# snap-research/3dgp

Hardware: AMD Instinct MI355X
Metric: generator-forward img/s @256^2, 64 steps (higher is better)
Workload: dtype f32; 1 GPU; BASELINE configs[2]: ImageNet 256x256, 64(+64) ray steps, cmax 512, c_dim 1000, tri-plane 512^2 x 96, full HIP path; batch_per_gpu=16, global_batch=16, img_resolution=256, num_ray_steps=64, depth_adaptor=False, parallelism=dp1 (batch-sharded, weights replicated)

## Files before the change

### 3dgp_amd/csrc/sampling.hip

```cpp
#include "common.h"

namespace {

constexpr int MAXS = 256;
constexpr int RAYS_PER_BLOCK = 4;
constexpr int MAXS_PASS = 512;
constexpr int MAXS_LONG = 1024;

template <int MS>
struct alignas(16) WaveScratchT {
    float z[MS];
    float sig[MS];
    float w[MS + 4];
    float cdf[MS];
    float bins[MS];
    float col[3][MS];
};
using WaveScratch = WaveScratchT<MAXS>;

template <int MS> struct alignas(16) MarchScratchT { float z[MS]; float sig[MS]; float w[MS + 4]; };
template <> struct alignas(16) MarchScratchT<MAXS> : WaveScratch {};
template <int MS> struct alignas(16) UnifyScratchT { float z[MS]; };
template <> struct alignas(16) UnifyScratchT<MAXS> : WaveScratch {};

__device__ __forceinline__ void wave_sync() {
    __builtin_amdgcn_fence(__ATOMIC_ACQ_REL, "wavefront");
    __builtin_amdgcn_wave_barrier();
}

__device__ __forceinline__ float s2t(float s, float t_near, float t_far) { return s * t_far + (1.0f - s) * t_near; }

template <bool LONGX>
__device__ __forceinline__ float exp_neg(float x) { return LONGX ? (float)exp(-(double)x) : expf(-x); }

template <bool LONGX = false>
__device__ void march_classical_lds(const float* z, const float* sig, float* w, int S, int flags, float cut_thr, float& final_T, float& wagg) {
    const int l = lane_id();
    double carry = 1.0;
    float wsum = 0.0f;
    if (S > 64 && S <= 128) {
        float alpha[2], fac[2];
#pragma unroll
        for (int c = 0; c < 2; c++) {
            const int i = 64 * c + l;
            alpha[c] = 0.f; fac[c] = 1.0f;
            if (i < S) {
                const float delta = (i < S - 1) ? (z[i + 1] - z[i]) : ((flags & 1) ? 1e10f : 1e-3f);
                float sp = (flags & 8) ? (sig[i] > 0.f ? sig[i] : 0.f) : softplus20f(sig[i]);
                if (sp < cut_thr) sp = 0.f;
                alpha[c] = 1.0f - exp_neg<LONGX>(delta * sp);
                fac[c] = (1.0f - alpha[c]) + 1e-10f;
            }
        }
        const double s0 = wave_scan_f64<true>((double)fac[0]), s1 = wave_scan_f64<true>((double)fac[1]);
        const double c1 = wave_last_f64(s0);
        const double i1 = s1 * c1;
        const float incl0 = (float)s0, incl1 = (float)i1;
        const float wi0 = alpha[0] * wave_shr1_f32(incl0, 1.0f), wi1 = alpha[1] * wave_shr1_f32(incl1, (float)c1);
        w[l] = wi0; wsum += wi0;
        if (64 + l < S) { w[64 + l] = wi1; wsum += wi1; }
        carry = wave_last_f64(i1);
    } else
    for (int base = 0; base < S; base += 64) {
        const int i = base + l;
        float alpha = 0.f, fac = 1.0f;
        if (i < S) {
            float delta = (i < S - 1) ? (z[i + 1] - z[i]) : ((flags & 1) ? 1e10f : 1e-3f);
            float sp = (flags & 8) ? (sig[i] > 0.f ? sig[i] : 0.f) : softplus20f(sig[i]);
            if (sp < cut_thr) sp = 0.f;
            alpha = 1.0f - exp_neg<LONGX>(delta * sp);
            fac = (1.0f - alpha) + 1e-10f;
        }
        const double incl64 = wave_scan_f64<true>((double)fac) * carry;
        const float incl = (float)incl64;
        const float excl = wave_shr1_f32(incl, (float)carry);
        const float wi = alpha * excl;
        if (i < S) { w[i] = wi; wsum += wi; }
        carry = wave_last_f64(incl64);
    }
    wagg = wave_sum_f32(wsum);
    final_T = (float)carry;
    wave_sync();
    if ((flags & 2) && l == 0) w[S - 1] += (1.0f - wagg);
    wave_sync();
}

template <bool LONGX = false>
__device__ void march_mip_lds(const float* z, const float* sig, float* w, int S, int flags, float density_bias, float cut_thr, float& final_T,
                              float& wagg) {
    const int l = lane_id();
    const int M = (flags & 1) ? S : S - 1;
    double carry = 1.0;
    float wsum = 0.0f;
    for (int base = 0; base < M; base += 64) {
        const int i = base + l;
        float alpha = 0.f, fac = 1.0f;
        if (i < M) {
            float delta, smid;
            if (i < S - 1) { delta = z[i + 1] - z[i]; smid = (sig[i] + sig[i + 1]) / 2.f; }
            else { delta = 1e10f; smid = sig[S - 1]; }
            float sp = softplus20f(smid + density_bias);
            if (sp < cut_thr) sp = 0.f;
            float dd = sp * delta;
            alpha = 1.0f - exp_neg<LONGX>(dd);
            fac = (1.0f - alpha) + 1e-10f;
        }
        const double incl64 = wave_scan_f64<true>((double)fac) * carry;
        const float incl = (float)incl64;
        const float excl = wave_shr1_f32(incl, (float)carry);
        const float wi = alpha * excl;
        if (i < M) { w[i] = wi; wsum += wi; }
        carry = wave_last_f64(incl64);
    }
    wagg = wave_sum_f32(wsum);
    final_T = (float)carry;
    wave_sync();
}

__device__ float torch_order_sum_lds(const float* w1, int n, float eps) {
    const int l = lane_id();
    if (n >= 8) {
        const int nv = n >> 3, nilp = nv >> 2;
        const int col = l & 7, a = (l >> 3) & 3;
        float acc = 0.f;
        for (int i = 0; i < nilp; i++) acc = __fadd_rn(acc, __fadd_rn(w1[(4 * i + a) * 8 + col], eps));
        for (int j = 4 * nilp; j < nv; j++) {
            const float v = __fadd_rn(w1[j * 8 + col], eps);
            if (a == 0) acc = __fadd_rn(acc, v);
        }
        float p = __shfl(acc, col, 64);
        p = __fadd_rn(p, __shfl(acc, col + 8, 64));
        p = __fadd_rn(p, __shfl(acc, col + 16, 64));
        p = __fadd_rn(p, __shfl(acc, col + 24, 64));
        float fin = 0.f;
        for (int k = nv * 8; k < n; k++) fin = __fadd_rn(fin, __fadd_rn(w1[k], eps));
#pragma unroll
        for (int c = 0; c < 8; c++) fin = __fadd_rn(fin, __int_as_float(__builtin_amdgcn_readlane(__float_as_int(p), c)));
        return fin;
    }
    float acc[4] = {0.f, 0.f, 0.f, 0.f};
    const int nilp = n >> 2;
    if (nilp)
        for (int k = 0; k < 4; k++) acc[k] = __fadd_rn(acc[k], __fadd_rn(w1[k], eps));
    for (int r = 4 * nilp; r < n; r++) acc[0] = __fadd_rn(acc[0], __fadd_rn(w1[r], eps));
    for (int k = 1; k < 4; k++) acc[0] = __fadd_rn(acc[0], acc[k]);
    return acc[0];
}

template <typename SC, typename GetU, typename Emit>
__device__ void importance_lds(SC& sc, int S, int Wn, GetU getu, int N, int mip, Emit emit) {
    const int l = lane_id();
    const float eps = 1e-5f;
    float* w = sc.w;
    constexpr int CAP = sizeof(sc.z) / sizeof(float), NV = (CAP > MAXS ? CAP : MAXS) / 64;
    if (mip) {
        float nv[NV];
#pragma unroll
        for (int c = 0; c < NV; c++) {
            const int i = l + 64 * c;
            if (i < Wn) {
                float a = (i - 1 >= 0) ? w[i - 1] : -INFINITY, b = w[i], d = (i + 1 < Wn) ? w[i + 1] : -INFINITY;
                float t0 = a > b ? a : b;
                float t1 = b > d ? b : d;
                nv[c] = (t0 + t1) / 2.f + 0.01f;
            }
        }
        wave_sync();
#pragma unroll
        for (int c = 0; c < NV; c++) {
            const int i = l + 64 * c;
            if (i < Wn) w[i] = nv[c];
        }
    } else {
        for (int i = l; i < Wn; i += 64) w[i] = w[i] + 1e-5f;
    }
    wave_sync();
    const int nb = S - 1, ns = Wn - 2, nc = ns + 1;
    for (int i = l; i < nb; i += 64) sc.bins[i] = 0.5f * (sc.z[i] + sc.z[i + 1]);
    const float totf = torch_order_sum_lds(w + 1, ns, eps);
    double carry = 0.0;
    if (l == 0) sc.cdf[0] = 0.f;
    for (int base = 0; base < ns; base += 64) {
        const int i = base + l;
        float pdf = (i < ns) ? (w[1 + i] + eps) / totf : 0.f;
        double incl = wave_scan_f64<false>((double)pdf) + carry;
        if (i < ns) sc.cdf[i + 1] = (float)incl;
        carry = wave_last_f64(incl);
    }
    wave_sync();
    for (int j = l; j < N; j += 64) {
        const float uu = getu(j);
        int lo = 0, hi = nc;
        while (lo < hi) {
            int mid = (lo + hi) >> 1;
            if (sc.cdf[mid] <= uu) lo = mid + 1; else hi = mid;
        }
        const int ind = lo;
        const int below = ind - 1 < 0 ? 0 : ind - 1;
        const int above = ind > ns ? ns : ind;
        const float cb = sc.cdf[below], ca = sc.cdf[above];
        const float bb = sc.bins[below < nb ? below : nb - 1], ba = sc.bins[above < nb ? above : nb - 1];
        float denom = ca - cb;
        if (denom < eps) denom = 1.f;
        const float smp = bb + (uu - cb) / denom * (ba - bb);
        emit(j, smp, ind, below, above);
    }
}

__device__ __forceinline__ float strat_one(float u, int k, int S, float step, int marcher) {
    auto lin = [&](int q) { return (S == 1) ? 0.f : ((q < S / 2) ? __fmaf_rn(step, (float)q, 0.f) : __fmaf_rn(-step, (float)(S - 1 - q), 1.f)); };
    if (marcher == 0) {
        const float lower = (k == 0) ? lin(0) : 0.5f * (lin(k) + lin(k - 1));
        const float upper = (k == S - 1) ? lin(S - 1) : 0.5f * (lin(k + 1) + lin(k));
        return lower + (upper - lower) * u;
    }
    const float delta = (float)((1.0 - 0.0) / (double)(S - 1));
    return lin(k) + u * delta;
}

__global__ __launch_bounds__(256) void stratified_kernel(const float* __restrict__ u, float* __restrict__ sdist, float* __restrict__ tdist,
                                                        int64_t n, int S, int marcher, float t_near, float t_far) {
    const float step = (1.f - 0.f) / (float)(S - 1);
    for (int64_t i = blockIdx.x * (int64_t)blockDim.x + threadIdx.x; i < n; i += (int64_t)gridDim.x * blockDim.x) {
        const float s = strat_one(u[i], (int)(i % S), S, step, marcher);
        sdist[i] = s;
        if (tdist) tdist[i] = s2t(s, t_near, t_far);
    }
}

__global__ __launch_bounds__(256) void stratified4_kernel(const float4* __restrict__ u, float4* __restrict__ sdist, float4* __restrict__ tdist,
                                                         int64_t n4, int S, int marcher, float t_near, float t_far) {
    const float step = (1.f - 0.f) / (float)(S - 1);
    const int S4 = S >> 2;
    for (int64_t i = blockIdx.x * (int64_t)blockDim.x + threadIdx.x; i < n4; i += (int64_t)gridDim.x * blockDim.x) {
        const int k = (int)(i % S4) * 4;
        const float4 uu = u[i];
        const float4 s = make_float4(strat_one(uu.x, k, S, step, marcher), strat_one(uu.y, k + 1, S, step, marcher), strat_one(uu.z, k + 2, S, step, marcher),
                                     strat_one(uu.w, k + 3, S, step, marcher));
        sdist[i] = s;
        if (tdist) tdist[i] = make_float4(s2t(s.x, t_near, t_far), s2t(s.y, t_near, t_far), s2t(s.z, t_near, t_far), s2t(s.w, t_near, t_far));
    }
}

__global__ __launch_bounds__(256) void density_activation_kernel(const float* __restrict__ x, float* __restrict__ y, int64_t n, int relu, float bias) {
    for (int64_t i = blockIdx.x * (int64_t)blockDim.x + threadIdx.x; i < n; i += (int64_t)gridDim.x * blockDim.x)
        y[i] = relu ? (x[i] > 0.f ? x[i] : 0.f) : softplus20f(x[i] + bias);
}

template <int MS>
__global__ __launch_bounds__(256) void ray_march_kernel(const float* __restrict__ colors, const float* __restrict__ dens,
                                                       const float* __restrict__ depths, float* __restrict__ rgb, float* __restrict__ depth_o,
                                                       float* __restrict__ weights, float* __restrict__ final_T, int64_t rays, int S, int C,
                                                       int marcher, int flags, float density_bias, float cut_thr) {
    __shared__ MarchScratchT<MS> scratch[RAYS_PER_BLOCK];
    const int wv = threadIdx.x >> 6, l = lane_id();
    const int64_t r = (int64_t)blockIdx.x * RAYS_PER_BLOCK + wv;
    if (r >= rays) return;
    MarchScratchT<MS>& sc = scratch[wv];
    for (int i = l; i < S; i += 64) { sc.z[i] = depths[r * S + i]; sc.sig[i] = dens[r * S + i]; }
    wave_sync();
    float fT, wagg;
    const int M = (marcher == 0) ? S : ((flags & 1) ? S : S - 1);
    if (MS > MAXS && S > MAXS) {
        if (marcher == 0) march_classical_lds<(MS > MAXS)>(sc.z, sc.sig, sc.w, S, flags, cut_thr, fT, wagg);
        else march_mip_lds<(MS > MAXS)>(sc.z, sc.sig, sc.w, S, flags, density_bias, cut_thr, fT, wagg);
    } else
    if (marcher == 0) march_classical_lds(sc.z, sc.sig, sc.w, S, flags, cut_thr, fT, wagg);
    else march_mip_lds(sc.z, sc.sig, sc.w, S, flags, density_bias, cut_thr, fT, wagg);
    if (weights) for (int i = l; i < M; i += 64) weights[r * M + i] = sc.w[i];
    for (int c = 0; c <= C; c++) {
        float acc = 0.0f;
        for (int i = l; i < M; i += 64) {
            float v;
            if (c < C) {
                v = colors[(r * S + i) * C + c];
                if (marcher == 1 && i < S - 1) v = (v + colors[(r * S + i + 1) * C + c]) / 2.f;
            } else {
                v = sc.z[i];
                if (marcher == 1 && i < S - 1) v = (v + sc.z[i + 1]) / 2.f;
            }
            acc += sc.w[i] * v;
        }
        float out = wave_sum_f32(acc);
        if (marcher == 1 && c < C) {
            if (flags & 4) out = out + 1.0f - wagg;
            out = out * 2.0f - 1.0f;
        }
        if (l == 0) { if (c < C) rgb[r * C + c] = out; else depth_o[r] = out; }
    }
    if (l == 0) final_T[r] = fT;
}

template <int MS>
__global__ __launch_bounds__(256) void sample_importance_kernel(const float* __restrict__ z, const float* __restrict__ weights,
                                                               const float* __restrict__ u, float* __restrict__ samples, int32_t* __restrict__ inds,
                                                               int32_t* __restrict__ below, int32_t* __restrict__ above, float* __restrict__ cdf_o,
                                                               int64_t rays, int S, int Wn, int N, int mip) {
    __shared__ WaveScratchT<MS> scratch[RAYS_PER_BLOCK];
    const int wv = threadIdx.x >> 6, l = lane_id();
    const int64_t r = (int64_t)blockIdx.x * RAYS_PER_BLOCK + wv;
    if (r >= rays) return;
    WaveScratchT<MS>& sc = scratch[wv];
    for (int i = l; i < S; i += 64) sc.z[i] = z[r * S + i];
    for (int i = l; i < Wn; i += 64) sc.w[i] = weights[r * Wn + i];
    wave_sync();
    importance_lds(sc, S, Wn, [&](int j) { return u[r * N + j]; }, N, mip, [&](int j, float smp, int ind, int bl, int ab) {
        samples[r * N + j] = smp;
        if (inds) { inds[r * N + j] = ind; below[r * N + j] = bl; above[r * N + j] = ab; }
    });
    if (cdf_o) for (int i = l; i < Wn - 1; i += 64) cdf_o[r * (Wn - 1) + i] = sc.cdf[i];
}

template <int NS>
__device__ __forceinline__ void stable_ranks_n(const float* key, int M, int* rank) {
    const int l = lane_id();
    float k[NS];
#pragma unroll
    for (int c = 0; c < NS; c++) { const int i = l + 64 * c; k[c] = i < M ? key[i] : 0.f; rank[c] = 0; }
#pragma unroll 4
    for (int m = 0; m < M; m++) {
        const float km = key[m];
#pragma unroll
        for (int c = 0; c < NS; c++) {
            const int i = l + 64 * c;
            rank[c] += (km < k[c] || (km == k[c] && m < i)) ? 1 : 0;
        }
    }
}
__device__ __forceinline__ void stable_ranks(const float* key, int M, int* rank ) {
#pragma unroll
    for (int c = 0; c < MAXS / 64; c++) rank[c] = 0;
    if (M <= 64) stable_ranks_n<1>(key, M, rank);
    else if (M <= 128) stable_ranks_n<2>(key, M, rank);
    else if (M <= 192) stable_ranks_n<3>(key, M, rank);
    else stable_ranks_n<4>(key, M, rank);
}

template <int NR>
__device__ __forceinline__ void stable_ranks_long(const float* key, int M, int (&rank)[NR]) {
    static_assert(NR == MAXS_PASS / 64 || NR == MAXS_LONG / 64, "stable_ranks_long: 8 or 16 slots");
#pragma unroll
    for (int c = 0; c < NR; c++) rank[c] = 0;
    if (M <= MAXS_PASS) stable_ranks_n<MAXS_PASS / 64>(key, M, rank);
    else stable_ranks_n<NR>(key, M, rank);
}

template <int NS, int CAP>
__device__ __forceinline__ void wave_bitonic_sort_n(float (&key)[CAP], int (&idx)[CAP]) {
    static_assert(NS <= CAP && (NS & (NS - 1)) == 0, "wave_bitonic_sort_n: NS a power of two within the arrays");
    const int l = lane_id();
#pragma unroll
    for (int k = 2; k <= 64 * NS; k <<= 1) {
#pragma unroll
        for (int j = k >> 1; j > 0; j >>= 1) {
            if (j >= 64) {
                const int js = j >> 6;
#pragma unroll
                for (int c = 0; c < NS; c++) {
                    if (c & js) continue;
                    const int c2 = c | js;
                    const bool asc = ((64 * c) & k) == 0;
                    const bool less2 = key[c2] < key[c] || (key[c2] == key[c] && idx[c2] < idx[c]);
                    if (less2 == asc) { const float tk = key[c]; key[c] = key[c2]; key[c2] = tk; const int ti = idx[c]; idx[c] = idx[c2]; idx[c2] = ti; }
                }
            } else {
#pragma unroll
                for (int c = 0; c < NS; c++) {
                    const float pk = __shfl_xor(key[c], j, 64);
                    const int pi = __shfl_xor(idx[c], j, 64);
                    const bool asc = ((64 * c + l) & k) == 0;
                    const bool keep_min = ((l & j) == 0) == asc;
                    const bool partner_less = pk < key[c] || (pk == key[c] && pi < idx[c]);
                    if (partner_less == keep_min) { key[c] = pk; idx[c] = pi; }
                }
            }
        }
    }
}

__device__ __forceinline__ void wave_bitonic_sort(float& key, int& idx) {
    const int l = lane_id();
#pragma unroll
    for (int k = 2; k <= 64; k <<= 1) {
#pragma unroll
        for (int j = k >> 1; j > 0; j >>= 1) {
            const float pk = __shfl_xor(key, j, 64);
            const int pi = __shfl_xor(idx, j, 64);
            const bool keep_min = ((l & j) == 0) == ((l & k) == 0);
            const bool partner_less = pk < key || (pk == key && pi < idx);
            if (partner_less == keep_min) { key = pk; idx = pi; }
        }
    }
}

__device__ __forceinline__ void wave_bitonic_sort2(float (&key)[2], int (&idx)[2]) {
    const int l = lane_id();
#pragma unroll
    for (int k = 2; k <= 128; k <<= 1) {
#pragma unroll
        for (int j = k >> 1; j > 0; j >>= 1) {
            if (j == 64) {
                const bool less1 = key[1] < key[0] || (key[1] == key[0] && idx[1] < idx[0]);
                if (less1) { const float tk = key[0]; key[0] = key[1]; key[1] = tk; const int ti = idx[0]; idx[0] = idx[1]; idx[1] = ti; }
            } else {
#pragma unroll
                for (int c = 0; c < 2; c++) {
                    const float pk = __shfl_xor(key[c], j, 64);
                    const int pi = __shfl_xor(idx[c], j, 64);
                    const bool asc = k == 128 ? true : (k == 64 ? c == 0 : ((l & k) == 0));
                    const bool keep_min = ((l & j) == 0) == asc;
                    const bool partner_less = pk < key[c] || (pk == key[c] && pi < idx[c]);
                    if (partner_less == keep_min) { key[c] = pk; idx[c] = pi; }
                }
            }
        }
    }
}

template <int MS>
__global__ __launch_bounds__(256) void importance_from_coarse_kernel(const float* __restrict__ rgbs, const float* __restrict__ sdist,
                                                                    const float* __restrict__ u_fine, float* __restrict__ tfine,
                                                                    float* __restrict__ sfine, int32_t* __restrict__ inds,
                                                                    int32_t* __restrict__ fine_perm, int64_t rays, int S, int N,
                                                                    int marcher, int flags, float density_bias, float cut_thr, float t_near, float t_far) {
    __shared__ WaveScratchT<MS> scratch[RAYS_PER_BLOCK];
    const int wv = threadIdx.x >> 6, l = lane_id();
    const int64_t r = (int64_t)blockIdx.x * RAYS_PER_BLOCK + wv;
    if (r >= rays) return;
    WaveScratchT<MS>& sc = scratch[wv];
    for (int i = l; i < S; i += 64) { sc.z[i] = sdist[r * S + i]; sc.sig[i] = rgbs[(r * S + i) * 4 + 3]; }
    float upre[MS / 64];
    if constexpr (MS > MAXS) {
        for (int i = l; i < N; i += 64) sc.col[1][i] = u_fine[r * N + i];
    } else {
#pragma unroll
    for (int c = 0; c < MS / 64; c++) upre[c] = (l + 64 * c < N) ? u_fine[r * N + l + 64 * c] : 0.f;
    }
    wave_sync();
    float fT, wagg;
    int Wn = S;
    if (MS > MAXS && S > MAXS) {
        if (marcher == 0) march_classical_lds<(MS > MAXS)>(sc.z, sc.sig, sc.w, S, flags, cut_thr, fT, wagg);
        else { march_mip_lds<(MS > MAXS)>(sc.z, sc.sig, sc.w, S, flags, density_bias, cut_thr, fT, wagg); Wn = (flags & 1) ? S : S - 1; }
    } else
    if (marcher == 0) march_classical_lds(sc.z, sc.sig, sc.w, S, flags, cut_thr, fT, wagg);
    else { march_mip_lds(sc.z, sc.sig, sc.w, S, flags, density_bias, cut_thr, fT, wagg); Wn = (flags & 1) ? S : S - 1; }
    float* tkey = sc.col[0];
    if constexpr (MS > MAXS)
        [[clang::always_inline]] importance_lds(sc, S, Wn, [&](int j) { return sc.col[1][j]; }, N, marcher, [&](int j, float smp, int ind, int, int) {
            tkey[j] = s2t(smp, t_near, t_far);
            if (sfine) sfine[r * N + j] = smp;
            if (inds) inds[r * N + j] = ind;
        });
    else
    importance_lds(sc, S, Wn, [&](int j) { float v = upre[0];
#pragma unroll
                                          for (int c = 1; c < MS / 64; c++) v = (j >> 6) == c ? upre[c] : v;
                                          return v; }, N, marcher, [&](int j, float smp, int ind, int, int) {
        tkey[j] = s2t(smp, t_near, t_far);
        if (sfine) sfine[r * N + j] = smp;
        if (inds) inds[r * N + j] = ind;
    });
    wave_sync();
    if (N <= 64) {
        float key = l < N ? tkey[l] : INFINITY;
        {
            if (l >= N) tkey[l] = INFINITY;
            wave_sync();
            int cnt = 0;
#pragma unroll
            for (int jj = 0; jj < 16; jj++) {
                const float4 k4 = *(const float4*)&tkey[4 * jj];
                cnt += (k4.x < key ? 1 : 0) + (k4.y < key ? 1 : 0) + (k4.z < key ? 1 : 0) + (k4.w < key ? 1 : 0);
            }
            int* slot = (int*)sc.bins;
            if (l < N) slot[cnt] = l;
            wave_sync();
            const bool mine = l >= N || slot[cnt] == l;
            if (__all(mine)) {
                if (l < N) {
                    const int src = slot[l];
                    tfine[r * N + l] = tkey[src];
                    if (fine_perm) fine_perm[r * N + l] = src;
                }
                return;
            }
        }
        int idx = l;
        wave_bitonic_sort(key, idx);
        if (l < N) {
            tfine[r * N + l] = key;
            if (fine_perm) fine_perm[r * N + l] = idx;
        }
        return;
    }
    if (N <= 128) {
        float key[2] = {tkey[l], l + 64 < N ? tkey[l + 64] : INFINITY};
        {
            if (l + 64 >= N) tkey[l + 64] = INFINITY;
            wave_sync();
            int cnt[2] = {0, 0};
#pragma unroll 8
            for (int jj = 0; jj < 32; jj++) {
                const float4 k4 = *(const float4*)&tkey[4 * jj];
#pragma unroll
                for (int c = 0; c < 2; c++)
                    cnt[c] += (k4.x < key[c] ? 1 : 0) + (k4.y < key[c] ? 1 : 0) + (k4.z < key[c] ? 1 : 0) + (k4.w < key[c] ? 1 : 0);
            }
            int* slot = (int*)sc.bins;
            slot[cnt[0]] = l;
            if (l + 64 < N) slot[cnt[1]] = l + 64;
            wave_sync();
            const bool mine = slot[cnt[0]] == l && (l + 64 >= N || slot[cnt[1]] == l + 64);
            if (__all(mine)) {
#pragma unroll
                for (int c = 0; c < 2; c++) {
                    const int pos = l + 64 * c;
                    if (pos < N) {
                        const int src = slot[pos];
                        tfine[r * N + pos] = tkey[src];
                        if (fine_perm) fine_perm[r * N + pos] = src;
                    }
                }
                return;
            }
        }
        int idx[2] = {l, l + 64};
        wave_bitonic_sort2(key, idx);
#pragma unroll
        for (int c = 0; c < 2; c++) {
            const int pos = l + 64 * c;
            if (pos < N) {
                tfine[r * N + pos] = key[c];
                if (fine_perm) fine_perm[r * N + pos] = idx[c];
            }
        }
        return;
    }
    if constexpr (MS > MAXS) {
        constexpr int NSL = MS / 64;
        float key[NSL];
        int idx[NSL];
#pragma unroll
        for (int c = 0; c < NSL; c++) { const int e = l + 64 * c; key[c] = e < N ? tkey[e] : INFINITY; idx[c] = e; }
        if (N <= 256) wave_bitonic_sort_n<4>(key, idx);
        else wave_bitonic_sort_n<NSL>(key, idx);
#pragma unroll
        for (int c = 0; c < NSL; c++) {
            const int pos = l + 64 * c;
            if (pos < N) {
                tfine[r * N + pos] = key[c];
                if (fine_perm) fine_perm[r * N + pos] = idx[c];
            }
        }
        return;
    } else {
    int rank[MAXS / 64];
    stable_ranks(tkey, N, rank);
#pragma unroll
    for (int c = 0; c < MAXS / 64; c++) {
        const int j = l + 64 * c;
        if (j < N) {
            tfine[r * N + rank[c]] = tkey[j];
            if (fine_perm) fine_perm[r * N + rank[c]] = j;
        }
    }
    }
}

template <int MS>
__global__ __launch_bounds__(256) void unify_kernel(const float* __restrict__ d1, const float* __restrict__ c1, const float* __restrict__ s1, int S1,
                                                   const float* __restrict__ d2, const float* __restrict__ c2, const float* __restrict__ s2, int S2,
                                                   float* __restrict__ d, float* __restrict__ c, float* __restrict__ s, int32_t* __restrict__ perm,
                                                   int64_t rays, int C) {
    __shared__ UnifyScratchT<MS> scratch[RAYS_PER_BLOCK];
    const int wv = threadIdx.x >> 6, l = lane_id();
    const int64_t r = (int64_t)blockIdx.x * RAYS_PER_BLOCK + wv;
    if (r >= rays) return;
    UnifyScratchT<MS>& sc = scratch[wv];
    const int M = S1 + S2;
    for (int i = l; i < M; i += 64) sc.z[i] = i < S1 ? d1[r * S1 + i] : d2[r * S2 + (i - S1)];
    wave_sync();
    int rank[MS / 64];
    if constexpr (MS > MAXS) stable_ranks_long(sc.z, M, rank);
    else stable_ranks(sc.z, M, rank);
#pragma unroll
    for (int cc = 0; cc < MS / 64; cc++) {
        const int i = l + 64 * cc;
        if (i >= M) continue;
        const int pos = rank[cc];
        d[r * M + pos] = sc.z[i];
        s[r * M + pos] = i < S1 ? s1[r * S1 + i] : s2[r * S2 + (i - S1)];
        for (int k = 0; k < C; k++) c[(r * M + pos) * C + k] = i < S1 ? c1[(r * S1 + i) * C + k] : c2[(r * S2 + (i - S1)) * C + k];
        if (perm) perm[r * M + pos] = i;
    }
}

template <int MS>
__global__ __launch_bounds__(256) void merge_composite_kernel(const float* __restrict__ rgbs1, const float* __restrict__ t1, int S1,
                                                             const float* __restrict__ rgbs2, const float* __restrict__ t2, int S2,
                                                             float* __restrict__ rgb, float* __restrict__ depth_o, float* __restrict__ wsum_o,
                                                             float* __restrict__ final_T, int32_t* __restrict__ perm, const int32_t* __restrict__ perm2, int64_t rays,
                                                             int marcher, int flags, float density_bias, float cut_thr) {
    __shared__ WaveScratchT<MS> scratch[RAYS_PER_BLOCK];
    const int wv = threadIdx.x >> 6, l = lane_id();
    const int64_t r = (int64_t)blockIdx.x * RAYS_PER_BLOCK + wv;
    if (r >= rays) return;
    WaveScratchT<MS>& sc = scratch[wv];
    const int M = S1 + S2;
    float4 cval[MS / 64];
#pragma unroll
    for (int cc = 0; cc < MS / 64; cc++) {
        const int i = l + 64 * cc;
        if (i < M) {
            sc.cdf[i] = i < S1 ? t1[r * S1 + i] : t2[r * S2 + (i - S1)];
            cval[cc] = i < S1 ? ((const float4*)rgbs1)[r * S1 + i] : ((const float4*)rgbs2)[r * S2 + (i - S1)];
        }
    }
    wave_sync();
    bool bad = false;
    for (int i = l; i < M; i += 64)
        if (i + 1 < M && i + 1 != S1 && sc.cdf[i + 1] < sc.cdf[i]) bad = true;
    constexpr int RK = (MS > MAXS ? MS : MAXS) / 64;
    int rank[RK];
    if (__any(bad)) {
        if constexpr (MS > MAXS) stable_ranks_long(sc.cdf, M, rank);
        else stable_ranks(sc.cdf, M, rank);
    } else {
        constexpr int NSL = MS / 64;
        float v[NSL];
        int lo[NSL], hi[NSL];
        bool fine[NSL];
        int* const last = (int*)sc.bins;
        for (int c = l; c <= S1 && c < MS; c += 64) last[c] = 0;
#pragma unroll
        for (int cc = 0; cc < NSL; cc++) {
            const int i = l + 64 * cc;
            v[cc] = i < M ? sc.cdf[i] : 0.f;
            fine[cc] = i >= S1 && i < M;
            lo[cc] = 0;
            hi[cc] = fine[cc] ? S1 : 0;
        }
        const int steps = 32 - __clz(S1);
        for (int it = 0; it < steps; it++) {
#pragma unroll
            for (int cc = 0; cc < NSL; cc++) {
                if (64 * cc + 64 <= S1) continue;
                const bool open = lo[cc] < hi[cc];
                const int mid = (lo[cc] + hi[cc]) >> 1;
                const float o = sc.cdf[open ? mid : 0];
                const bool right = o <= v[cc];
                lo[cc] = (open && right) ? mid + 1 : lo[cc];
                hi[cc] = (open && !right) ? mid : hi[cc];
            }
        }
        wave_sync();
#pragma unroll
        for (int cc = 0; cc < NSL; cc++) {
            const int i = l + 64 * cc;
            if (fine[cc]) atomicMax(&last[lo[cc]], i - S1 + 1);
        }
        wave_sync();
#pragma unroll
        for (int cc = 0; cc < RK; cc++) rank[cc] = 0;
        int carry = 0;
#pragma unroll
        for (int cc = 0; cc < NSL; cc++) {
            const int i = l + 64 * cc;
            if (64 * cc < S1) {
                const int incl = max(wave_scan_max_i32((i <= S1 && i < MS) ? last[i] : 0), carry);
                carry = wave_last_i32(incl);
                rank[cc] = fine[cc] ? (i - S1) + lo[cc] : i + incl;
            } else {
                rank[cc] = (i - S1) + lo[cc];
            }
        }
    }
#pragma unroll
    for (int cc = 0; cc < MS / 64; cc++) {
        const int i = l + 64 * cc;
        if (i >= M) continue;
        const int pos = rank[cc];
        const float4 v = cval[cc];
        sc.z[pos] = sc.cdf[i];
        sc.col[0][pos] = v.x; sc.col[1][pos] = v.y; sc.col[2][pos] = v.z; sc.sig[pos] = v.w;
        if (perm) perm[r * M + pos] = i < S1 ? i : S1 + (perm2 ? perm2[r * S2 + (i - S1)] : i - S1);
    }
    wave_sync();
    float fT, wagg;
    const int Mm = (marcher == 0) ? M : ((flags & 1) ? M : M - 1);
    if (MS > MAXS && M > MAXS) {
        if (marcher == 0) march_classical_lds<(MS > MAXS)>(sc.z, sc.sig, sc.w, M, flags, cut_thr, fT, wagg);
        else march_mip_lds<(MS > MAXS)>(sc.z, sc.sig, sc.w, M, flags, density_bias, cut_thr, fT, wagg);
    } else
    if (marcher == 0) march_classical_lds(sc.z, sc.sig, sc.w, M, flags, cut_thr, fT, wagg);
    else march_mip_lds(sc.z, sc.sig, sc.w, M, flags, density_bias, cut_thr, fT, wagg);
    float acc[4] = {0.f, 0.f, 0.f, 0.f}, wacc = 0.f;
    for (int i = l; i < Mm; i += 64) {
        const float wi = sc.w[i];
        wacc += wi;
#pragma unroll
        for (int c = 0; c < 4; c++) {
            float v = c < 3 ? sc.col[c][i] : sc.z[i];
            if (marcher == 1 && i < M - 1) v = (v + (c < 3 ? sc.col[c][i + 1] : sc.z[i + 1])) / 2.f;
            acc[c] += wi * v;
        }
    }
    float out[4];
#pragma unroll
    for (int c = 0; c < 4; c++) out[c] = wave_sum_f32(acc[c]);
    const float wtot = wave_sum_f32(wacc);
    if (marcher == 1) {
#pragma unroll
        for (int c = 0; c < 3; c++) {
            if (flags & 4) out[c] = out[c] + 1.0f - wagg;
            out[c] = out[c] * 2.0f - 1.0f;
        }
    }
    if (l == 0) {
        rgb[r * 3 + 0] = out[0]; rgb[r * 3 + 1] = out[1]; rgb[r * 3 + 2] = out[2];
        depth_o[r] = out[3];
        if (wsum_o) wsum_o[r] = wtot;
        if (final_T) final_T[r] = fT;
    }
}

inline int ray_blocks(int64_t rays) { return (int)cdiv64(rays, RAYS_PER_BLOCK); }

}

TDGP_API int tdgp_sample_stratified(const float* u, float* sdist, float* tdist, int64_t rays, int S, int marcher, float t_near,
                                    float t_far, tdgp_stream_t stream) {
    TDGP_CHECK(u && sdist, TDGP_EINVAL, "sample_stratified: null pointer");
    TDGP_CHECK(S >= 2 && rays >= 0, TDGP_EINVAL, "sample_stratified: need S >= 2");
    TDGP_CHECK(marcher == 0 || marcher == 1, TDGP_EINVAL, "sample_stratified: unknown ray marcher %d", marcher);
    const int64_t n = rays * S;
    if (n == 0) return TDGP_OK;
    if ((S & 3) == 0 && (((uintptr_t)u | (uintptr_t)sdist | (uintptr_t)tdist) & 15) == 0) {
        TDGP_LAUNCH("stratified_kernel", stratified4_kernel, dim3((int)min((int64_t)8192, cdiv64(n / 4, 256))), dim3(256), 0, (hipStream_t)stream, (const float4*)u,
                    (float4*)sdist, (float4*)tdist, n / 4, S, marcher, t_near, t_far);
        TDGP_LAUNCH_CHECK();
        return TDGP_OK;
    }
    TDGP_LAUNCH("stratified_kernel", stratified_kernel, dim3((int)min((int64_t)8192, cdiv64(n, 256))), dim3(256), 0, (hipStream_t)stream, u, sdist, tdist, n, S,
                       marcher, t_near, t_far);
    TDGP_LAUNCH_CHECK();
    return TDGP_OK;
}

TDGP_API int tdgp_density_activation(const float* sigma, float* out, int64_t n, int flags, float density_bias, tdgp_stream_t stream) {
    TDGP_CHECK(sigma && out, TDGP_EINVAL, "density_activation: null pointer");
    TDGP_CHECK(n >= 0, TDGP_EINVAL, "density_activation: negative length");
    if (n == 0) return TDGP_OK;
    TDGP_LAUNCH("density_activation_kernel", density_activation_kernel, dim3((int)min((int64_t)8192, cdiv64(n, 256))), dim3(256), 0, (hipStream_t)stream, sigma, out, n,
                (flags & 8) ? 1 : 0, density_bias);
    TDGP_LAUNCH_CHECK();
    return TDGP_OK;
}

TDGP_API int tdgp_ray_march(const float* colors, const float* densities, const float* depths, float* rgb, float* depth, float* weights,
                            float* final_T, int64_t rays, int S, int C, int marcher, int flags, float density_bias, float cut_threshold, tdgp_stream_t stream) {
    TDGP_CHECK(colors && densities && depths && rgb && depth && final_T, TDGP_EINVAL, "ray_march: null pointer");
    TDGP_CHECK(S >= 2 && S <= MAXS_LONG, TDGP_EUNSUPPORTED, "ray_march: S=%d outside [2,%d] (a merged list of at most %d + %d samples)", S, MAXS_LONG,
               MAXS_PASS, MAXS_PASS);
    TDGP_CHECK(C >= 1 && C <= 8, TDGP_EUNSUPPORTED, "ray_march: C=%d outside [1,8]", C);
    TDGP_CHECK(marcher == 0 || marcher == 1, TDGP_EINVAL, "ray_march: unknown ray marcher %d", marcher);
    TDGP_FAULT_CHECK("ray_march");
    if (rays == 0) return TDGP_OK;
    if (S <= MAXS)
        TDGP_LAUNCH("ray_march_kernel", ray_march_kernel<MAXS>, dim3(ray_blocks(rays)), dim3(256), 0, (hipStream_t)stream, colors, densities, depths, rgb, depth, weights,
                    final_T, rays, S, C, marcher, flags, density_bias, cut_threshold);
    else
        TDGP_LAUNCH("ray_march_kernel", ray_march_kernel<MAXS_LONG>, dim3(ray_blocks(rays)), dim3(256), 0, (hipStream_t)stream, colors, densities, depths, rgb, depth,
                    weights, final_T, rays, S, C, marcher, flags, density_bias, cut_threshold);
    TDGP_LAUNCH_CHECK();
    return TDGP_OK;
}

TDGP_API int tdgp_sample_importance(const float* z, const float* weights, const float* u, float* samples, int32_t* inds, int32_t* below,
                                    int32_t* above, float* cdf, int64_t rays, int S, int Wn, int N, int marcher, tdgp_stream_t stream) {
    TDGP_CHECK(z && weights && u && samples, TDGP_EINVAL, "sample_importance: null pointer");
    TDGP_CHECK(!inds || (below && above), TDGP_EINVAL, "sample_importance: inds/below/above come together");
    TDGP_CHECK(S >= 4 && S <= MAXS_PASS && Wn >= 3 && Wn <= S && N >= 1, TDGP_EUNSUPPORTED,
               "sample_importance: bad S=%d Wn=%d N=%d (S at most %d: beyond it torch's sum order is not restated)", S, Wn, N, MAXS_PASS);
    if (rays == 0) return TDGP_OK;
    if (S <= MAXS)
        TDGP_LAUNCH("sample_importance_kernel", sample_importance_kernel<MAXS>, dim3(ray_blocks(rays)), dim3(256), 0, (hipStream_t)stream, z, weights, u, samples, inds,
                    below, above, cdf, rays, S, Wn, N, marcher);
    else
        TDGP_LAUNCH("sample_importance_kernel", sample_importance_kernel<MAXS_PASS>, dim3(ray_blocks(rays)), dim3(256), 0, (hipStream_t)stream, z, weights, u, samples,
                    inds, below, above, cdf, rays, S, Wn, N, marcher);
    TDGP_LAUNCH_CHECK();
    return TDGP_OK;
}

TDGP_API int tdgp_unify_samples(const float* d1, const float* c1, const float* s1, int S1, const float* d2, const float* c2, const float* s2,
                                int S2, float* d, float* c, float* s, int32_t* perm, int64_t rays, int C, tdgp_stream_t stream) {
    TDGP_CHECK(d1 && c1 && s1 && d2 && c2 && s2 && d && c && s, TDGP_EINVAL, "unify_samples: null pointer");
    TDGP_CHECK(S1 >= 1 && S2 >= 1 && S1 + S2 <= MAXS_LONG, TDGP_EUNSUPPORTED, "unify_samples: S1+S2=%d > %d", S1 + S2, MAXS_LONG);
    if (rays == 0) return TDGP_OK;
    if (S1 + S2 <= MAXS)
        TDGP_LAUNCH("unify_kernel", unify_kernel<MAXS>, dim3(ray_blocks(rays)), dim3(256), 0, (hipStream_t)stream, d1, c1, s1, S1, d2, c2, s2, S2, d, c, s, perm, rays, C);
    else
        TDGP_LAUNCH("unify_kernel", unify_kernel<MAXS_LONG>, dim3(ray_blocks(rays)), dim3(256), 0, (hipStream_t)stream, d1, c1, s1, S1, d2, c2, s2, S2, d, c, s, perm, rays,
                    C);
    TDGP_LAUNCH_CHECK();
    return TDGP_OK;
}

TDGP_API int tdgp_importance_from_coarse(const float* rgbs_coarse, const float* sdist, const float* u_fine, float* tdist_fine,
                                         float* sdist_fine, int32_t* inds, int32_t* fine_perm, int64_t rays, int S, int N, int marcher, int flags,
                                         float density_bias, float cut_threshold, float t_near, float t_far, tdgp_stream_t stream) {
    TDGP_CHECK(rgbs_coarse && sdist && u_fine && tdist_fine, TDGP_EINVAL, "importance_from_coarse: null pointer");
    TDGP_CHECK(S >= 4 && S <= MAXS_PASS && N >= 1 && N <= MAXS_PASS, TDGP_EUNSUPPORTED, "importance_from_coarse: bad S=%d N=%d (both at most %d)", S, N, MAXS_PASS);
    TDGP_CHECK(marcher == 0 || marcher == 1, TDGP_EINVAL, "importance_from_coarse: unknown ray marcher %d", marcher);
    TDGP_FAULT_CHECK("importance_from_coarse");
    if (rays == 0) return TDGP_OK;
    if (S <= 128 && N <= 128)
        TDGP_LAUNCH("importance_from_coarse_kernel", importance_from_coarse_kernel<128>, dim3(ray_blocks(rays)), dim3(256), 0, (hipStream_t)stream, rgbs_coarse, sdist,
                           u_fine, tdist_fine, sdist_fine, inds, fine_perm, rays, S, N, marcher, flags, density_bias, cut_threshold, t_near, t_far);
    else if (S <= MAXS && N <= MAXS)
        TDGP_LAUNCH("importance_from_coarse_kernel", importance_from_coarse_kernel<MAXS>, dim3(ray_blocks(rays)), dim3(256), 0, (hipStream_t)stream, rgbs_coarse, sdist,
                           u_fine, tdist_fine, sdist_fine, inds, fine_perm, rays, S, N, marcher, flags, density_bias, cut_threshold, t_near, t_far);
    else
        TDGP_LAUNCH("importance_from_coarse_kernel", importance_from_coarse_kernel<MAXS_PASS>, dim3(ray_blocks(rays)), dim3(256), 0, (hipStream_t)stream, rgbs_coarse,
                    sdist, u_fine, tdist_fine, sdist_fine, inds, fine_perm, rays, S, N, marcher, flags, density_bias, cut_threshold, t_near, t_far);
    TDGP_LAUNCH_CHECK();
    return TDGP_OK;
}

TDGP_API int tdgp_merge_composite(const float* rgbs_coarse, const float* t_coarse, int S1, const float* rgbs_fine, const float* t_fine, int S2,
                                  float* rgb, float* depth, float* wsum, float* final_T, int32_t* perm, const int32_t* fine_perm, int64_t rays,
                                  int marcher, int flags, float density_bias, float cut_threshold, tdgp_stream_t stream) {
    TDGP_CHECK(rgbs_coarse && t_coarse && rgbs_fine && t_fine && rgb && depth, TDGP_EINVAL, "merge_composite: null pointer");
    TDGP_CHECK(S1 >= 1 && S2 >= 1 && S1 + S2 <= MAXS_LONG, TDGP_EUNSUPPORTED, "merge_composite: S1+S2=%d > %d", S1 + S2, MAXS_LONG);
    TDGP_CHECK(marcher == 0 || marcher == 1, TDGP_EINVAL, "merge_composite: unknown ray marcher %d", marcher);
    TDGP_FAULT_CHECK("merge_composite");
    if (rays == 0) return TDGP_OK;
    if (S1 + S2 <= 128)
        TDGP_LAUNCH("merge_composite_kernel", merge_composite_kernel<128>, dim3(ray_blocks(rays)), dim3(256), 0, (hipStream_t)stream, rgbs_coarse, t_coarse, S1,
                           rgbs_fine, t_fine, S2, rgb, depth, wsum, final_T, perm, fine_perm, rays, marcher, flags, density_bias, cut_threshold);
    else if (S1 + S2 <= 192)
        TDGP_LAUNCH("merge_composite_kernel", merge_composite_kernel<192>, dim3(ray_blocks(rays)), dim3(256), 0, (hipStream_t)stream, rgbs_coarse, t_coarse, S1,
                           rgbs_fine, t_fine, S2, rgb, depth, wsum, final_T, perm, fine_perm, rays, marcher, flags, density_bias, cut_threshold);
    else if (S1 + S2 <= MAXS)
        TDGP_LAUNCH("merge_composite_kernel", merge_composite_kernel<MAXS>, dim3(ray_blocks(rays)), dim3(256), 0, (hipStream_t)stream, rgbs_coarse, t_coarse, S1,
                           rgbs_fine, t_fine, S2, rgb, depth, wsum, final_T, perm, fine_perm, rays, marcher, flags, density_bias, cut_threshold);
    else if (S1 + S2 <= MAXS_PASS)
        TDGP_LAUNCH("merge_composite_kernel", merge_composite_kernel<MAXS_PASS>, dim3(ray_blocks(rays)), dim3(256), 0, (hipStream_t)stream, rgbs_coarse, t_coarse, S1,
                    rgbs_fine, t_fine, S2, rgb, depth, wsum, final_T, perm, fine_perm, rays, marcher, flags, density_bias, cut_threshold);
    else
        TDGP_LAUNCH("merge_composite_kernel", merge_composite_kernel<MAXS_LONG>, dim3(ray_blocks(rays)), dim3(256), 0, (hipStream_t)stream, rgbs_coarse, t_coarse, S1,
                    rgbs_fine, t_fine, S2, rgb, depth, wsum, final_T, perm, fine_perm, rays, marcher, flags, density_bias, cut_threshold);
    TDGP_LAUNCH_CHECK();
    return TDGP_OK;
}
```

Baseline: 731.1 img/s.

## Add two-rays-per-wave specialized kernels for 64+64 importance sampling and merge

Adds kernels specialised for S=N=64 (and S1=S2=64) in which each wavefront handles two rays at once. The per-ray steps (load, march, CDF, search, sort-by-count, merge-rank, composite) are interleaved so the latency of one ray's independent instructions overlaps the other's. The kernels use fixed-size LDS scratch and a counting-rank fast path, falling back to bitonic sort or stable ranks when that fails. This raises work per wave and LDS use per block, which may reduce occupancy.

```diff
diff --git a/3dgp_amd/csrc/sampling.hip b/3dgp_amd/csrc/sampling.hip
--- a/3dgp_amd/csrc/sampling.hip
+++ b/3dgp_amd/csrc/sampling.hip
@@ -725,7 +725,386 @@
     }
 }
 
+constexpr int PAIR_RAYS_PER_BLOCK = 8;
+
+__device__ __forceinline__ void classical_alpha(const float* z, const float* sig, int i, int S, int flags, float cut_thr, float& alpha, float& fac) {
+    const float delta = (i < S - 1) ? (z[i + 1] - z[i]) : ((flags & 1) ? 1e10f : 1e-3f);
+    float sp = (flags & 8) ? (sig[i] > 0.f ? sig[i] : 0.f) : softplus20f(sig[i]);
+    if (sp < cut_thr) sp = 0.f;
+    alpha = 1.0f - expf(-(delta * sp));
+    fac = (1.0f - alpha) + 1e-10f;
+}
+__device__ __forceinline__ void mip_alpha(const float* z, const float* sig, int i, int S, int M, float density_bias, float cut_thr, float& alpha, float& fac) {
+    alpha = 0.f; fac = 1.0f;
+    if (i < M) {
+        float delta, smid;
+        if (i < S - 1) { delta = z[i + 1] - z[i]; smid = (sig[i] + sig[i + 1]) / 2.f; }
+        else { delta = 1e10f; smid = sig[S - 1]; }
+        float sp = softplus20f(smid + density_bias);
+        if (sp < cut_thr) sp = 0.f;
+        const float dd = sp * delta;
+        alpha = 1.0f - expf(-dd);
+        fac = (1.0f - alpha) + 1e-10f;
+    }
+}
+
+struct alignas(16) ImpPairScratch { float z[64]; float sig[64]; float w[64 + 4]; float cdf[64]; float bins[64]; float key[64]; };
+
+struct ImpRay {
+    ImpPairScratch* sc;
+    int64_t r;
+    bool live;
+    float zl, sg, u;
+    float nv;
+    float key;
+    int cnt, idx;
+};
+
+__device__ __forceinline__ void imp_load(ImpRay& R, const float* __restrict__ rgbs, const float* __restrict__ sdist, const float* __restrict__ u_fine) {
+    const int l = lane_id();
+    R.zl = sdist[R.r * 64 + l]; R.sg = rgbs[(R.r * 64 + l) * 4 + 3]; R.u = u_fine[R.r * 64 + l];
+}
+__device__ __forceinline__ void imp_park(ImpRay& R) { const int l = lane_id(); R.sc->z[l] = R.zl; R.sc->sig[l] = R.sg; }
+__device__ __forceinline__ float imp_march(ImpRay& R, int marcher, int flags, float density_bias, float cut_thr) {
+    const int l = lane_id();
+    const int M = (marcher == 0 || (flags & 1)) ? 64 : 63;
+    float alpha, fac;
+    if (marcher == 0) classical_alpha(R.sc->z, R.sc->sig, l, 64, flags, cut_thr, alpha, fac);
+    else mip_alpha(R.sc->z, R.sc->sig, l, 64, M, density_bias, cut_thr, alpha, fac);
+    const double carry = 1.0;
+    const double incl64 = wave_scan_f64<true>((double)fac) * carry;
+    const float incl = (float)incl64;
+    const float excl = wave_shr1_f32(incl, (float)carry);
+    const float wi = alpha * excl;
+    float wsum = 0.0f;
+    if (l < M) { R.sc->w[l] = wi; wsum += wi; }
+    return wave_sum_f32(wsum);
+}
+__device__ __forceinline__ void imp_last_back(ImpRay& R, float wagg) { if (lane_id() == 0) R.sc->w[63] += (1.0f - wagg); }
+__device__ __forceinline__ void imp_smooth_read(ImpRay& R, int Wn) {
+    const int i = lane_id();
+    const float* w = R.sc->w;
+    if (i < Wn) {
+        const float a = (i - 1 >= 0) ? w[i - 1] : -INFINITY, b = w[i], d = (i + 1 < Wn) ? w[i + 1] : -INFINITY;
+        const float t0 = a > b ? a : b, t1 = b > d ? b : d;
+        R.nv = (t0 + t1) / 2.f + 0.01f;
+    }
+}
+__device__ __forceinline__ void imp_smooth_write(ImpRay& R, int Wn) { const int i = lane_id(); if (i < Wn) R.sc->w[i] = R.nv; }
+__device__ __forceinline__ void imp_offset(ImpRay& R, int Wn) { const int i = lane_id(); if (i < Wn) R.sc->w[i] = R.sc->w[i] + 1e-5f; }
+__device__ __forceinline__ float torch_order_sum_62(const float* w1, int n, float eps) {
+    const int l = lane_id();
+    const int col = l & 7, a = (l >> 3) & 3;
+    float acc = 0.f;
+    acc = __fadd_rn(acc, __fadd_rn(w1[a * 8 + col], eps));
+#pragma unroll
+    for (int j = 4; j < 7; j++) {
+        const float v = __fadd_rn(w1[j * 8 + col], eps);
+        if (a == 0) acc = __fadd_rn(acc, v);
+    }
+    float p = __shfl(acc, col, 64);
+    p = __fadd_rn(p, __shfl(acc, col + 8, 64));
+    p = __fadd_rn(p, __shfl(acc, col + 16, 64));
+    p = __fadd_rn(p, __shfl(acc, col + 24, 64));
+    float fin = 0.f;
+#pragma unroll
+    for (int k = 56; k < 62; k++) {
+        const float t = __fadd_rn(fin, __fadd_rn(w1[k], eps));
+        fin = k < n ? t : fin;
+    }
+#pragma unroll
+    for (int c = 0; c < 8; c++) fin = __fadd_rn(fin, __int_as_float(__builtin_amdgcn_readlane(__float_as_int(p), c)));
+    return fin;
+}
+__device__ __forceinline__ void imp_cdf(ImpRay& R, int Wn) {
+    const int l = lane_id();
+    const float eps = 1e-5f;
+    ImpPairScratch& sc = *R.sc;
+    const int ns = Wn - 2;
+    if (l < 63) sc.bins[l] = 0.5f * (sc.z[l] + sc.z[l + 1]);
+    const float totf = torch_order_sum_62(sc.w + 1, ns, eps);
+    const double carry = 0.0;
+    if (l == 0) sc.cdf[0] = 0.f;
+    const float pdf = (l < ns) ? (sc.w[1 + l] + eps) / totf : 0.f;
+    const double incl = wave_scan_f64<false>((double)pdf) + carry;
+    if (l < ns) sc.cdf[l + 1] = (float)incl;
+}
+__device__ __forceinline__ void imp_search(ImpRay& R, int Wn, float t_near, float t_far, float* __restrict__ sfine, int32_t* __restrict__ inds) {
+    const int l = lane_id();
+    const float eps = 1e-5f;
+    ImpPairScratch& sc = *R.sc;
+    const int nb = 63, ns = Wn - 2, nc = ns + 1;
+    const float uu = R.u;
+    int lo = 0, hi = nc;
+#pragma unroll
+    for (int it = 0; it < 6; it++) {
+        const bool open = lo < hi;
+        const int mid = (lo + hi) >> 1;
+        const bool right = sc.cdf[open ? mid : 0] <= uu;
+        lo = (open && right) ? mid + 1 : lo;
+        hi = (open && !right) ? mid : hi;
+    }
+    const int ind = lo;
+    const int below = ind - 1 < 0 ? 0 : ind - 1;
+    const int above = ind > ns ? ns : ind;
+    const float cb = sc.cdf[below], ca = sc.cdf[above];
+    const float bb = sc.bins[below < nb ? below : nb - 1], ba = sc.bins[above < nb ? above : nb - 1];
+    float denom = ca - cb;
+    if (denom < eps) denom = 1.f;
+    const float smp = bb + (uu - cb) / denom * (ba - bb);
+    R.key = s2t(smp, t_near, t_far);
+    sc.key[l] = R.key;
+    if (R.live) {
+        if (sfine) sfine[R.r * 64 + l] = smp;
+        if (inds) inds[R.r * 64 + l] = ind;
+    }
+}
+__device__ __forceinline__ void imp_count(ImpRay& R) {
+    const int l = lane_id();
+    int cnt = 0;
+#pragma unroll
+    for (int jj = 0; jj < 16; jj++) {
+        const float4 k4 = *(const float4*)&R.sc->key[4 * jj];
+        cnt += (k4.x < R.key ? 1 : 0) + (k4.y < R.key ? 1 : 0) + (k4.z < R.key ? 1 : 0) + (k4.w < R.key ? 1 : 0);
+    }
+    R.cnt = cnt;
+    ((int*)R.sc->bins)[cnt] = l;
+}
+__device__ __forceinline__ bool imp_gather(ImpRay& R) {
+    const int l = lane_id();
+    const int* slot = (const int*)R.sc->bins;
+    const bool ok = __all(slot[R.cnt] == l);
+    const int src = ok ? slot[l] : l;
+    R.key = R.sc->key[src];
+    R.idx = src;
+    return ok;
+}
+__device__ __forceinline__ void imp_store(const ImpRay& R, float* __restrict__ tfine, int32_t* __restrict__ fine_perm) {
+    const int l = lane_id();
+    if (R.live) {
+        tfine[R.r * 64 + l] = R.key;
+        if (fine_perm) fine_perm[R.r * 64 + l] = R.idx;
+    }
+}
+
+__global__ __launch_bounds__(256, 8) void importance_from_coarse_pair_kernel(const float* __restrict__ rgbs, const float* __restrict__ sdist,
+                                                                            const float* __restrict__ u_fine, float* __restrict__ tfine,
+                                                                            float* __restrict__ sfine, int32_t* __restrict__ inds,
+                                                                            int32_t* __restrict__ fine_perm, int64_t rays, int marcher, int flags,
+                                                                            float density_bias, float cut_thr, float t_near, float t_far) {
+    __shared__ ImpPairScratch scratch[PAIR_RAYS_PER_BLOCK];
+    const int wv = threadIdx.x >> 6;
+    const int64_t r0 = ((int64_t)blockIdx.x * (PAIR_RAYS_PER_BLOCK / 2) + wv) * 2;
+    if (r0 >= rays) return;
+    ImpRay A, B;
+    A.sc = &scratch[2 * wv]; A.r = r0; A.live = true;
+    B.sc = &scratch[2 * wv + 1]; B.live = r0 + 1 < rays; B.r = B.live ? r0 + 1 : r0;
+    imp_load(A, rgbs, sdist, u_fine); imp_load(B, rgbs, sdist, u_fine);
+    imp_park(A); imp_park(B);
+    wave_sync();
+    const float waA = imp_march(A, marcher, flags, density_bias, cut_thr), waB = imp_march(B, marcher, flags, density_bias, cut_thr);
+    wave_sync();
+    int Wn = 64;
+    if (marcher == 0) {
+        if (flags & 2) { imp_last_back(A, waA); imp_last_back(B, waB); }
+        wave_sync();
+        imp_offset(A, Wn); imp_offset(B, Wn);
+    } else {
+        Wn = (flags & 1) ? 64 : 63;
+        imp_smooth_read(A, Wn); imp_smooth_read(B, Wn);
+        wave_sync();
+        imp_smooth_write(A, Wn); imp_smooth_write(B, Wn);
+    }
+    wave_sync();
+    imp_cdf(A, Wn); imp_cdf(B, Wn);
+    wave_sync();
+    imp_search(A, Wn, t_near, t_far, sfine, inds); imp_search(B, Wn, t_near, t_far, sfine, inds);
+    wave_sync();
+    imp_count(A); imp_count(B);
+    wave_sync();
+    const bool okA = imp_gather(A), okB = imp_gather(B);
+    if (!okA) wave_bitonic_sort(A.key, A.idx);
+    if (!okB) wave_bitonic_sort(B.key, B.idx);
+    imp_store(A, tfine, fine_perm); imp_store(B, tfine, fine_perm);
+}
+
+struct alignas(16) MergePairScratch {
+    float key[128];
+    float z[128];
+    float sig[128];
+    float col[3][128];
+};
+
+struct MergeRay {
+    MergePairScratch* sc;
+    int64_t r;
+    bool live;
+    float k[2];
+    float4 c[2];
+    int p2;
+    int lo;
+    int rank[2];
+    bool bad;
+};
+
+__device__ __forceinline__ void mrg_load(MergeRay& R, const float* __restrict__ rgbs1, const float* __restrict__ t1, const float* __restrict__ rgbs2,
+                                         const float* __restrict__ t2, const int32_t* __restrict__ perm2, bool want_perm) {
+    const int l = lane_id();
+    R.k[0] = t1[R.r * 64 + l]; R.k[1] = t2[R.r * 64 + l];
+    R.c[0] = ((const float4*)rgbs1)[R.r * 64 + l]; R.c[1] = ((const float4*)rgbs2)[R.r * 64 + l];
+    R.p2 = (want_perm && perm2) ? perm2[R.r * 64 + l] : l;
+}
+__device__ __forceinline__ void mrg_park(MergeRay& R) { const int l = lane_id(); R.sc->key[l] = R.k[0]; R.sc->key[64 + l] = R.k[1]; }
+__device__ __forceinline__ void mrg_search(MergeRay& R) {
+    const int l = lane_id();
+    const float* key = R.sc->key;
+    R.bad = l < 63 && (key[l + 1] < key[l] || key[64 + l + 1] < key[64 + l]);
+    int* const last = (int*)R.sc->z;
+    last[l] = 0;
+    if (l == 0) last[64] = 0;
+    const float v = R.k[1];
+    int lo = 0, hi = 64;
+#pragma unroll
+    for (int it = 0; it < 7; it++) {
+        const bool open = lo < hi;
+        const int mid = (lo + hi) >> 1;
+        const bool right = key[open ? mid : 0] <= v;
+        lo = (open && right) ? mid + 1 : lo;
+        hi = (open && !right) ? mid : hi;
+    }
+    R.lo = lo;
+}
+__device__ __forceinline__ void mrg_scatter_last(MergeRay& R) { atomicMax(&((int*)R.sc->z)[R.lo], lane_id() + 1); }
+__device__ __forceinline__ bool mrg_ranks(MergeRay& R) {
+    const int l = lane_id();
+    const int incl = max(wave_scan_max_i32(((const int*)R.sc->z)[l]), 0);
+    R.rank[0] = l + incl;
+    R.rank[1] = l + R.lo;
+    return __any(R.bad);
+}
+__device__ __forceinline__ void mrg_scatter(MergeRay& R, int32_t* __restrict__ perm) {
+    const int l = lane_id();
+    MergePairScratch& sc = *R.sc;
+#pragma unroll
+    for (int cc = 0; cc < 2; cc++) {
+        const int pos = R.rank[cc];
+        const float4 v = R.c[cc];
+        sc.z[pos] = R.k[cc];
+        sc.col[0][pos] = v.x; sc.col[1][pos] = v.y; sc.col[2][pos] = v.z; sc.sig[pos] = v.w;
+        if (perm && R.live) perm[R.r * 128 + pos] = cc == 0 ? l : 64 + R.p2;
+    }
+}
+__device__ __forceinline__ void mrg_march(MergeRay& R, int marcher, int flags, float density_bias, float cut_thr, float& final_T, float& wagg) {
+    const int l = lane_id();
+    MergePairScratch& sc = *R.sc;
+    float* w = sc.key;
+    double carry = 1.0;
+    float wsum = 0.0f;
+    if (marcher == 0) {
+        float alpha[2], fac[2];
+#pragma unroll
+        for (int c = 0; c < 2; c++) classical_alpha(sc.z, sc.sig, 64 * c + l, 128, flags, cut_thr, alpha[c], fac[c]);
+        const double s0 = wave_scan_f64<true>((double)fac[0]), s1 = wave_scan_f64<true>((double)fac[1]);
+        const double c1 = wave_last_f64(s0);
+        const double i1 = s1 * c1;
+        const float incl0 = (float)s0, incl1 = (float)i1;
+        const float wi0 = alpha[0] * wave_shr1_f32(incl0, 1.0f), wi1 = alpha[1] * wave_shr1_f32(incl1, (float)c1);
+        w[l] = wi0; wsum += wi0;
+        w[64 + l] = wi1; wsum += wi1;
+        carry = wave_last_f64(i1);
+    } else {
+        const int M = (flags & 1) ? 128 : 127;
+#pragma unroll
+        for (int base = 0; base < 128; base += 64) {
+            const int i = base + l;
+            float alpha, fac;
+            mip_alpha(sc.z, sc.sig, i, 128, M, density_bias, cut_thr, alpha, fac);
+            const double incl64 = wave_scan_f64<true>((double)fac) * carry;
+            const float incl = (float)incl64;
+            const float excl = wave_shr1_f32(incl, (float)carry);
+            const float wi = alpha * excl;
+            if (i < M) { w[i] = wi; wsum += wi; }
+            carry = wave_last_f64(incl64);
+        }
+    }
+    wagg = wave_sum_f32(wsum);
+    final_T = (float)carry;
+}
+__device__ __forceinline__ void mrg_last_back(MergeRay& R, float wagg) { if (lane_id() == 0) R.sc->key[127] += (1.0f - wagg); }
+__device__ __forceinline__ void mrg_composite(MergeRay& R, int marcher, int flags, float wagg, float fT, float* __restrict__ rgb, float* __restrict__ depth_o,
+                                              float* __restrict__ wsum_o, float* __restrict__ final_T) {
+    const int l = lane_id();
+    const MergePairScratch& sc = *R.sc;
+    const float* w = sc.key;
+    const int Mm = (marcher == 0 || (flags & 1)) ? 128 : 127;
+    float acc[4] = {0.f, 0.f, 0.f, 0.f}, wacc = 0.f;
+#pragma unroll
+    for (int i = l; i < 128; i += 64) {
+        if (i < Mm) {
+            const float wi = w[i];
+            wacc += wi;
+#pragma unroll
+            for (int c = 0; c < 4; c++) {
+                float v = c < 3 ? sc.col[c][i] : sc.z[i];
+                if (marcher == 1 && i < 127) v = (v + (c < 3 ? sc.col[c][i + 1] : sc.z[i + 1])) / 2.f;
+                acc[c] += wi * v;
+            }
+        }
+    }
+    float out[4];
+#pragma unroll
+    for (int c = 0; c < 4; c++) out[c] = wave_sum_f32(acc[c]);
+    const float wtot = wave_sum_f32(wacc);
+    if (marcher == 1) {
+#pragma unroll
+        for (int c = 0; c < 3; c++) {
+            if (flags & 4) out[c] = out[c] + 1.0f - wagg;
+            out[c] = out[c] * 2.0f - 1.0f;
+        }
+    }
+    if (l == 0 && R.live) {
+        rgb[R.r * 3 + 0] = out[0]; rgb[R.r * 3 + 1] = out[1]; rgb[R.r * 3 + 2] = out[2];
+        depth_o[R.r] = out[3];
+        if (wsum_o) wsum_o[R.r] = wtot;
+        if (final_T) final_T[R.r] = fT;
+    }
+}
+
+__global__ __launch_bounds__(256, 8) void merge_composite_pair_kernel(const float* __restrict__ rgbs1, const float* __restrict__ t1,
+                                                                     const float* __restrict__ rgbs2, const float* __restrict__ t2,
+                                                                     float* __restrict__ rgb, float* __restrict__ depth_o, float* __restrict__ wsum_o,
+                                                                     float* __restrict__ final_T, int32_t* __restrict__ perm, const int32_t* __restrict__ perm2,
+                                                                     int64_t rays, int marcher, int flags, float density_bias, float cut_thr) {
+    __shared__ MergePairScratch scratch[PAIR_RAYS_PER_BLOCK];
+    const int wv = threadIdx.x >> 6;
+    const int64_t r0 = ((int64_t)blockIdx.x * (PAIR_RAYS_PER_BLOCK / 2) + wv) * 2;
+    if (r0 >= rays) return;
+    MergeRay A, B;
+    A.sc = &scratch[2 * wv]; A.r = r0; A.live = true;
+    B.sc = &scratch[2 * wv + 1]; B.live = r0 + 1 < rays; B.r = B.live ? r0 + 1 : r0;
+    mrg_load(A, rgbs1, t1, rgbs2, t2, perm2, perm != nullptr); mrg_load(B, rgbs1, t1, rgbs2, t2, perm2, perm != nullptr);
+    mrg_park(A); mrg_park(B);
+    wave_sync();
+    mrg_search(A); mrg_search(B);
+    wave_sync();
+    mrg_scatter_last(A); mrg_scatter_last(B);
+    wave_sync();
+    const bool slowA = mrg_ranks(A), slowB = mrg_ranks(B);
+    if (slowA) stable_ranks_n<2>(A.sc->key, 128, A.rank);
+    if (slowB) stable_ranks_n<2>(B.sc->key, 128, B.rank);
+    wave_sync();
+    mrg_scatter(A, perm); mrg_scatter(B, perm);
+    wave_sync();
+    float fTA, waA, fTB, waB;
+    mrg_march(A, marcher, flags, density_bias, cut_thr, fTA, waA); mrg_march(B, marcher, flags, density_bias, cut_thr, fTB, waB);
+    wave_sync();
+    if (marcher == 0 && (flags & 2)) { mrg_last_back(A, waA); mrg_last_back(B, waB); }
+    wave_sync();
+    mrg_composite(A, marcher, flags, waA, fTA, rgb, depth_o, wsum_o, final_T); mrg_composite(B, marcher, flags, waB, fTB, rgb, depth_o, wsum_o, final_T);
+}
+
 inline int ray_blocks(int64_t rays) { return (int)cdiv64(rays, RAYS_PER_BLOCK); }
+inline int pair_blocks(int64_t rays) { return (int)cdiv64(rays, PAIR_RAYS_PER_BLOCK); }
 
 }
 
@@ -816,7 +1195,10 @@
     TDGP_CHECK(marcher == 0 || marcher == 1, TDGP_EINVAL, "importance_from_coarse: unknown ray marcher %d", marcher);
     TDGP_FAULT_CHECK("importance_from_coarse");
     if (rays == 0) return TDGP_OK;
-    if (S <= 128 && N <= 128)
+    if (S == 64 && N == 64)
+        TDGP_LAUNCH("importance_from_coarse_kernel", importance_from_coarse_pair_kernel, dim3(pair_blocks(rays)), dim3(256), 0, (hipStream_t)stream, rgbs_coarse, sdist,
+                    u_fine, tdist_fine, sdist_fine, inds, fine_perm, rays, marcher, flags, density_bias, cut_threshold, t_near, t_far);
+    else if (S <= 128 && N <= 128)
         TDGP_LAUNCH("importance_from_coarse_kernel", importance_from_coarse_kernel<128>, dim3(ray_blocks(rays)), dim3(256), 0, (hipStream_t)stream, rgbs_coarse, sdist,
                            u_fine, tdist_fine, sdist_fine, inds, fine_perm, rays, S, N, marcher, flags, density_bias, cut_threshold, t_near, t_far);
     else if (S <= MAXS && N <= MAXS)
@@ -837,7 +1219,10 @@
     TDGP_CHECK(marcher == 0 || marcher == 1, TDGP_EINVAL, "merge_composite: unknown ray marcher %d", marcher);
     TDGP_FAULT_CHECK("merge_composite");
     if (rays == 0) return TDGP_OK;
-    if (S1 + S2 <= 128)
+    if (S1 == 64 && S2 == 64)
+        TDGP_LAUNCH("merge_composite_kernel", merge_composite_pair_kernel, dim3(pair_blocks(rays)), dim3(256), 0, (hipStream_t)stream, rgbs_coarse, t_coarse, rgbs_fine,
+                    t_fine, rgb, depth, wsum, final_T, perm, fine_perm, rays, marcher, flags, density_bias, cut_threshold);
+    else if (S1 + S2 <= 128)
         TDGP_LAUNCH("merge_composite_kernel", merge_composite_kernel<128>, dim3(ray_blocks(rays)), dim3(256), 0, (hipStream_t)stream, rgbs_coarse, t_coarse, S1,
                            rgbs_fine, t_fine, S2, rgb, depth, wsum, final_T, perm, fine_perm, rays, marcher, flags, density_bias, cut_threshold);
     else if (S1 + S2 <= 192)
```

Result: faster. 744.2 img/s, median of 6 (+1.8%).
